# bronemos/view-fusion

Measured on AMD Instinct MI355X. Metric: denoise_steps_per_sec, higher is better.
Workload: dtype f32; 1 GPU; small UNet 64x64 (33.9M params), B=16/GPU N=6 (S=96 views/GPU), training iteration fwd+bwd+Adam, linear T=2000 schedule; global_batch=16, views=6, parallelism=dp1, launch=HIP-graph replay of the whole iteration

## Files before the change

include/vf_hip.h:

```cpp
#ifndef VF_HIP_H
#define VF_HIP_H
#ifdef __cplusplus
extern "C" {
#endif

int vf_gn_fwd(const float* x, const float* gamma, const float* beta, float* y, float* mean ,
              float* rstd , int S, int C, int HW, int groups, float eps, int silu, void* stream);
int vf_gn_bwd_emits_rowsum(int C, int HW, int groups);
int vf_gn_plan(int C, int HW, int groups, int cat, int C1, int has_addend, int has_addend2, int has_dx2, int* out );
int vf_gn_bwd(const float* x, const float* gamma, const float* beta, const float* mean, const float* rstd,
              const float* dy, const float* addend, float* dx, float* dgamma_part, float* dbeta_part,
              float* dx_rowsum, int S, int C, int HW, int groups, int silu, void* stream);
int vf_gn_cat_fwd(const float* x, const float* x2, int C1, const float* gamma, const float* beta, float* y, float* mean,
                  float* rstd, int S, int C, int HW, int groups, float eps, int silu, void* stream);
int vf_gn_cat_bwd(const float* x, const float* x2, int C1, const float* gamma, const float* beta, const float* mean,
                  const float* rstd, const float* dy, const float* addend, const float* addend2, float* dx, float* dx2,
                  float* dgamma_part, float* dbeta_part, float* dx_rowsum, int S, int C, int HW, int groups, int silu,
                  void* stream);
int vf_rowsum(const float* x, float* out , int rows, int len, void* stream);
int vf_bias_grad(const float* dy, float* db, float* dvb, int S, int C, int HW, void* stream);
int vf_colsum(const float* part , float* out , int batch, int S, int C,
              void* stream);
int vf_colsum_multi(const void* desc, int n, long total_blocks, void* stream);

// ... 39 lines not shown
                         long ws_floats, int S, int Cin, int Cout, int H, int W, void* stream);
long vf_conv1x1_bf16x3_pack_dwords(int M, int K);
int vf_conv1x1_bf16x3_pack(const float* w_oihw, void* w3_fwd, void* w3_bwd, int Cout, int Cin, void* stream);
int vf_conv1x1_bf16x3(const float* x, const float* x2, int C1in, const void* w3, const float* bias,
                      const float* view_bias, const float* residual, float* y, float* y2, int C1out, int S, int Cin,
                      int Cout, int HW, void* stream);
long vf_conv_wgrad_ws_floats(int S, int Cin, int Cout, int H, int W, int KS);
int vf_conv_wgrad(const float* x, const float* dy, float* dw_oihw, float* ws, long ws_floats, int S, int Cin,
                  int Cout, int H, int W, int KS, int mode, void* stream);
int vf_conv_wgrad_main(const float* x, const float* dy, float* dw_oihw, float* ws, long ws_floats, int S, int Cin,
                       int Cout, int H, int W, int KS, int mode, long long* desc9, int* nblocks, void* stream);
int vf_conv1x1_cat_wgrad_main(const float* x1, const float* x2, int C1, const float* dy, float* dw_oihw, float* ws,
                              long ws_floats, int S, int Cin, int Cout, int H, int W, long long* desc9, int* nblocks,
                              void* stream);
int vf_sumpool2(const float* x, float* y, long n_out, int Wo, void* stream);

int vf_wino_supported(int H, int W, int mode);
int vf_wino_pack_sizes(int Cout, int Cin, long* fwd_floats, long* bwd_floats);
int vf_wino_pack_weights(const float* w_oihw, float* u_fwd, float* u_bwd , int Cout, int Cin,
                         void* stream);
int vf_wino_pack_weights_multi(const void* desc, int nlayers, long total_blocks, void* stream);
long vf_wino_conv_ws_floats(int S, int Cin, int Cout, int H, int W);
int vf_wino_conv_fill_pct(int S, int Cin, int Cout, int H, int W, int* tiles_out);
int vf_wino_conv_fwd(const float* x, const float* u_packed, const float* bias, const float* view_bias,
                     const float* residual, float* y, float* ws, long ws_floats, int S, int Cin, int Cout, int H,
                     int W, int mode, void* stream);
int vf_wino_conv_gn_fusable(int S, int Cin, int Cout, int H, int W, int mode, int groups);
int vf_wino_conv_fwd_gn(const float* x, const float* u_packed, const float* bias , const float* view_bias ,
                        const float* residual , float* y, int store_y, const float* gn_gamma, const float* gn_beta,
                        float* a_out, int groups, float eps, int silu, float* ws, long ws_floats, int S, int Cin, int Cout,
// ... 272 lines not shown
```

view_fusion_amd/_lib.py:

```python
import ctypes
import os

import torch

_HERE = os.path.dirname(os.path.abspath(__file__))
LIB_PATH = os.path.join(_HERE, "lib", "libvf_hip.so")
_OVERRIDE = os.environ.get("VF_HIP_LIB") if os.environ.get("VF_DEBUG_AB") == "1" else None
if _OVERRIDE:
    LIB_PATH = _OVERRIDE
elif os.environ.get("VF_HIP_LIB"):
    import warnings
    warnings.warn("VF_HIP_LIB is ignored unless VF_DEBUG_AB=1 (kernel-tuning aid)", stacklevel=2)

_P, _I, _L, _F = ctypes.c_void_p, ctypes.c_int, ctypes.c_long, ctypes.c_float
_U64 = ctypes.c_uint64

SIGNATURES = {
    "vf_gn_fwd": [_P, _P, _P, _P, _P, _P, _I, _I, _I, _I, _F, _I, _P],
    "vf_gn_bwd_emits_rowsum": [_I, _I, _I],
    "vf_gn_plan": [_I, _I, _I, _I, _I, _I, _I, _I, _P],
    "vf_gn_cat_fwd": [_P, _P, _I, _P, _P, _P, _P, _P, _I, _I, _I, _I, _F, _I, _P],
    "vf_gn_cat_bwd": [_P, _P, _I, _P, _P, _P, _P, _P, _P, _P, _P, _P, _P, _P, _P, _I, _I, _I, _I, _I, _P],
    "vf_conv1x1_cat_fwd": [_P, _P, _I, _P, _P, _P, _P, _L, _I, _I, _I, _I, _I, _P],
    "vf_conv1x1_cat_dgrad": [_P, _P, _P, _P, _I, _I, _I, _I, _I, _I, _P],
# ... 28 lines not shown
    "vf_wino44_pack_sizes": [_I, _I, ctypes.POINTER(_L), ctypes.POINTER(_L)],
    "vf_wino44_pack_weights": [_P, _P, _P, _I, _I, _P],
    "vf_wino44_pack_weights_multi": [_P, _I, _L, _P],
    "vf_wino44_conv_ws_floats": [_I, _I, _I, _I, _I],
    "vf_wino44_conv_fill_pct": [_I, _I, _I, _I, _I, ctypes.POINTER(_I)],
    "vf_wino44_conv_fwd": [_P, _P, _P, _P, _P, _P, _P, _L, _I, _I, _I, _I, _I, _I, _P],
    "vf_wino_conv_plan": [_I, _I, _I, _I, _I, _I, _I, _I, _L, _P],
    "vf_wino_wgrad_ws_floats": [_I, _I, _I, _I, _I],
    "vf_wino_wgrad_supported": [_I, _I, _I],
    "vf_wino_wgrad": [_P, _P, _P, _P, _P, _P, _L, _I, _I, _I, _I, _I, _I, _P],
    "vf_wino_wgrad_main": [_P, _P, _P, _P, _P, _P, _L, _I, _I, _I, _I, _I, _I, _P, _P, _P],
    "vf_wino44_reduce_multi": [_P, _I, _I, _P],
    "vf_conv_wgrad_main": [_P, _P, _P, _P, _L, _I, _I, _I, _I, _I, _I, _I, _P, _P, _P],
    "vf_conv1x1_cat_wgrad_main": [_P, _P, _I, _P, _P, _P, _L, _I, _I, _I, _I, _I, _P, _P, _P],
    "vf_sumpool2": [_P, _P, _L, _I, _P],
    "vf_time_affine_fwd": [_P, _I, _P, _P, _I, _I, _I, _P],
    "vf_time_affine_ws_floats": [_I, _I],
    "vf_time_affine_bwd": [_P, _I, _P, _P, _P, _P, _P, _P, _P, _I, _I, _I, _P],
    "vf_bgemm": [_P, _P, _P, _P, _I, _I, _I, _I, _L, _L, _L, _L, _L, _L, _L, _L, _L, _F, _F, _P],
    "vf_attention_fwd": [_P, _P, _P, _I, _I, _I, _P],
    "vf_attention_fwd_kernel": [_I, _I, _I],
    "vf_attention_dscore": [_P, _P, _P, _P, _P, _I, _I, _I, _P],
    "vf_attention_dvdk": [_P, _P, _P, _P, _P, _I, _I, _I, _P],
    "vf_attn_stream_fwd": [_P, _P, _P, _I, _I, _I, _P],
    "vf_attn_stream_bwd": [_P, _P, _P, _P, _P, _P, _I, _I, _I, _P],
    "vf_attn_stream_plan": [_P, _P, _I, _I, _I, _P],
    "vf_softmax_fwd": [_P, _P, _I, _I, _P],
    "vf_softmax_bwd": [_P, _P, _P, _I, _I, _P],
    "vf_bgemm_plan": [_P, _P, _I, _I, _I, _I, _L, _L, _L, _L, _L, _L, _L, _P],
    "vf_softmax_plan": [_I, _I, _P],
# ... 83 lines not shown
    "vf_distill_target": [_P, _P, _P, _P, _P, _P, _P, _P, _P, _P, _P, _P, _P, _P, _I, _I, _I, _I, _P, _P],
    "vf_distill_step_host": [_U64, _P, _I, _P, _I],
    "vf_loss_weights_trunc_snr_host": [_P, _I, _I, _P],
    "vf_stack_views_sc": [_P, _P, _P, _P, _P, _P, _P, _P, _P, _P, _P, _I, _I, _I, _I, _I, _I, _I, _P],
    "vf_draw_self_cond": [_U64, _P, ctypes.c_uint, _P, _I, _P],
    "vf_self_cond_estimate": [_P, _P, _P, _P, _L, _L, _I, _P, _P, _I, _I, _I, _I, _I, _P],
    "vf_self_cond_draw_host": [_U64, _P, ctypes.c_uint, _P, _I],
    "vf_self_cond_coeffs_host": [_P, _I, _P, _P, _I],
    "vf_rng_host_philox": [_P, _P, _P],
    "vf_rng_host_normal": [_U64, _P, _I, _I, _P, _I, _I],
    "vf_rng_host_train_scalars": [_U64, _P, _I, _P, _P, _I],
    "vf_batch_assemble": [_P, _L, _I, _I, _U64, _P, _P, _I, _I, _I, _I, _P, _P, _P, _P, _P],
    "vf_batch_host_plan": [_U64, _P, _I, _I, _I, _I, _L, _P, _P, _P, _P, _P, _P, _P],
}
_RESTYPE = {"vf_conv1x1_bf16x3_pack_dwords": _L, "vf_conv_wgrad_ws_floats": _L, "vf_time_affine_ws_floats": _L, "vf_wino_conv_ws_floats": _L, "vf_wino44_conv_ws_floats": _L, "vf_wino_wgrad_ws_floats": _L, "vf_conv_fwd_ws_floats": _L,
            "vf_conv_small_pack_floats": _L, "vf_ssim_workspace_floats": _L, "vf_lpips_workspace_floats": _L}

_lib = None
N_CALLS = 0


class VFHipError(RuntimeError):
    pass


def load():
    global _lib
    if _lib is None:
        if not os.path.exists(LIB_PATH):
            raise VFHipError(
                f"{LIB_PATH} not found: build it with `python -m view_fusion_amd.build` "
# ... 23 lines not shown
```

view_fusion_amd/ops/conv.py:

```python
import ctypes

import torch

from .. import _lib, reducer
from .state import st
from .bf16x3 import _packed_b3, _use_b3
from .core import _MODES, _c, _call, _check, _launch, _ptr, _stream, _workspace
from .deferred import _defer_begin, _gout, _rowsum_get, _rowsum_put, _wred_ws
from .norm import group_norm
from .packing import _WINO_ABI, _conv_ws, _packed, _packed_small, _packed_wino, _wino_ws
from .policy import use_small_conv, use_winograd, use_winograd_wgrad, wino_kind


def _wgrad(entry, front, back, need, owners, keep, generic, flops, tag, strm):
    dev = keep[0].device
    ws = _wred_ws(dev, need) if (st.WRED_DEFER and (st.WRED_DEFER_GENERIC or not generic)
                                 and _defer_begin(owners, st.slab_sums)) else None
    if ws is None:
        ws = _workspace(dev, need)
        _launch("conv_wgrad", flops, entry, *front, _ptr(ws), ws.numel(), *back, strm, tag=tag)
        return False
    row, nblk = (ctypes.c_longlong * 9)(), ctypes.c_int(0)
    _launch("conv_wgrad", flops, entry + "_main", *front, _ptr(ws), ws.numel(), *back, ctypes.cast(row, ctypes.c_void_p),
            ctypes.cast(ctypes.pointer(nblk), ctypes.c_void_p), strm, tag=tag)
    st.slab_sums.add(dev, (list(row), nblk.value, (ws, *keep)))
    return True


def _conv_small(x, x2, weight, bias, view_bias, residual, S, Cin, Cout, H, W, KS, m):
    wd = weight.detach()
    _check(wd)
    y = torch.empty(S, Cout, H, W, device=x.device, dtype=torch.float32)
    wp = _packed_small(weight) if KS == 3 else None
    if wp is not None:
        _launch("conv_fwd", 2.0 * S * Cout * Cin * 9 * H * W, "vf_conv_small_gn", _ptr(x), None, 0, _ptr(wd), _ptr(bias),
                _ptr(view_bias), _ptr(residual), _ptr(y), S, Cin, Cout, H, W, 3, None, None, None, 0, 1e-5, 0, None, None,
                None, 0, 0, None, None, _ptr(wp), m, _stream(), tag=(Cin, Cout, H, KS, m))
        return y
    _launch("conv_fwd", 2.0 * S * Cout * Cin * KS * KS * H * W, "vf_conv_small", _ptr(x), _ptr(x2),
            x.shape[1] if x2 is not None else 0, _ptr(wd), _ptr(bias), _ptr(view_bias), _ptr(residual), _ptr(y), S, Cin,
            Cout, H, W, KS, m, _stream(), tag=(Cin, Cout, H, KS, m))
# ... 28 lines not shown
        _check(x, bias, view_bias, residual)
        ctx.tap = tap
        if tap:
            ctx.set_materialize_grads(False)
        S, Cin, Hi, Wi = x.shape
        Cout, _, KS, _ = weight.shape
        m = _MODES[mode]
        if m == 1 and (Hi % 2 or Wi % 2):
            raise ValueError(f"stride-2 conv on a {Hi}x{Wi} map: both sides must be even")
        H, W = (Hi // 2, Wi // 2) if m == 1 else ((Hi * 2, Wi * 2) if m == 2 else (Hi, Wi))
        y = torch.empty(S, Cout, H, W, device=x.device, dtype=torch.float32)
        flops = 2.0 * S * Cout * Cin * KS * KS * H * W
        nb = 4.0 * (x.numel() + y.numel() + weight.numel() + (residual.numel() if residual is not None else 0))
        wino = wino_kind(S, Cin, Cout, H, W, KS, m, train=bool(training))
        ctx.b3 = _use_b3(KS, m, H * W)
        if ctx.b3:
            wf, wb = _packed_b3(layer, force=training)
            _launch("conv_fwd", flops, "vf_conv1x1_bf16x3", _ptr(x), None, 0, ctypes.c_void_p(wf.data_ptr()), _ptr(bias),
                    _ptr(view_bias), _ptr(residual), _ptr(y), None, 0, S, Cin, Cout, H * W, _stream(),
                    tag=(Cin, Cout, H, KS, m))
        elif wino:
            wf, wb = _packed_wino(layer, training, wino)
            ws, nws = _wino_ws(x.device, S, Cin, Cout, H, W, wino)
            _launch("conv_fwd", flops, _WINO_ABI[wino][3], _ptr(x), _ptr(wf), _ptr(bias), _ptr(view_bias),
                    _ptr(residual), _ptr(y), _ptr(ws), nws, S, Cin, Cout, H, W, m, _stream(),
                    tag=(Cin, Cout, H, KS, m), nbytes=nb)
        else:
            wf, wb = _packed(layer, force=training)
            ws, nws = _conv_ws(x.device, S, Cin, Cout, H, W, KS)
            _launch("conv_fwd", flops, "vf_conv_fwd", _ptr(x), _ptr(wf), _ptr(bias), _ptr(view_bias),
                    _ptr(residual), _ptr(y), _ptr(ws), nws, S, Cin, Cout, H, W, KS, m, _stream(),
# ... 4 lines not shown
        ctx.wb, ctx.m, ctx.KS, ctx.Cout = wb, m, KS, Cout
        ctx.has = (bias is not None, view_bias is not None, residual is not None)
        ctx.pw, ctx.pb, ctx.twin = weight, bias, (twin.bias if twin is not None else None)
        return (y, x.view_as(x)) if tap else y

    @staticmethod
    def backward(ctx, dy, dtap=None):
        (x,) = ctx.saved_tensors
        dy = _c(dy)
        dtap = _c(dtap) if dtap is not None else None
        S, Cin, Hi, Wi = x.shape
        _, Cout, H, W = dy.shape
        KS, m = ctx.KS, ctx.m
        strm = _stream()
        dx = dw = db = dvb = dres = None
        if ctx.needs_input_grad[0] and ctx.wino:
            dfull = torch.empty(S, Cin, H, W, device=x.device, dtype=torch.float32)
            ws, nws = _wino_ws(x.device, S, Cout, Cin, H, W, ctx.wino)
            _launch("conv_dgrad", ctx.flops, _WINO_ABI[ctx.wino][3], _ptr(dy), _ptr(ctx.wb), None, None, None,
                    _ptr(dfull), _ptr(ws), nws, S, Cout, Cin, H, W, 0, strm, tag=ctx.tag,
                    nbytes=4.0 * (dy.numel() + dfull.numel() + ctx.pw.numel()))
            if m == 2:
                dx = torch.empty_like(x)
                _call("vf_sumpool2", _ptr(dfull), _ptr(dx), dx.numel(), Wi, strm)
            else:
                dx = dfull
        elif ctx.needs_input_grad[0] and ctx.b3:
            dx = torch.empty_like(x)
            _launch("conv_dgrad", ctx.flops, "vf_conv1x1_bf16x3", _ptr(dy), None, 0, ctypes.c_void_p(ctx.wb.data_ptr()), None,
                    None, None, _ptr(dx), None, 0, S, Cout, Cin, H * W, strm, tag=ctx.tag)
        elif ctx.needs_input_grad[0]:
# ... 8 lines not shown
                        None, 0, S, Cout, Cin, H, W, KS, 4, strm, tag=ctx.tag)
                dtap = None
            else:
                dup = torch.empty(S, Cin, H, W, device=x.device, dtype=torch.float32)
                _launch("conv_dgrad", ctx.flops, "vf_conv_fwd", _ptr(dy), _ptr(ctx.wb), None, None, None, _ptr(dup),
                        None, 0, S, Cout, Cin, H, W, KS, 0, strm, tag=ctx.tag)
                dx = torch.empty_like(x)
                _call("vf_sumpool2", _ptr(dup), _ptr(dx), dx.numel(), Wi, strm)
        hb, hv, hr = ctx.has
        want_b, want_v = hb and ctx.needs_input_grad[2], hv and ctx.needs_input_grad[3]
        arena = reducer.ACTIVE is not None
        hit = _rowsum_get(dy) if (want_b or want_v) else None
        if hit is not None:
            dvb, db = hit[1], (hit[2].view_as(hit[2]) if hit[2] is not None else None)
        db2 = None
        if ctx.needs_input_grad[1] and use_winograd_wgrad(S, Cin, Cout, H, W, KS, m):
            need = _lib.load().vf_wino_wgrad_ws_floats(S, Cin, Cout, H, W)
            dw = _gout(ctx.pw, Cout, Cin, 3, 3, like=x)
            db_here = None
            if want_b and db is None:
                db = db_here = _gout(ctx.pb, Cout, like=x)
                if hr:
                    db2 = _gout(ctx.twin, Cout, like=x)
            owners = [ctx.pw] + ([ctx.pb] if db_here is not None else []) + \
                     ([ctx.twin] if (db2 is not None and ctx.twin is not None) else [])
            if _wgrad("vf_wino_wgrad", (_ptr(x), _ptr(dy), _ptr(dw), _ptr(db_here), _ptr(db2)), (S, Cin, Cout, H, W, m),
                      need, owners, (dw, db_here, db2), False, ctx.flops, ctx.tag, strm):
                dw = dw.view_as(dw)
                if db_here is not None:
                    db = db_here.view_as(db_here)
        elif ctx.needs_input_grad[1]:
# ... 159 lines not shown
```

view_fusion_amd/ops/state.py:

```python
import os


class State:
    def __init__(self):
        self.KERNEL_LOG = None
        self._KIND_OVERRIDE = None
        self.WINOGRAD = True
        self.FORCE_WINOGRAD = False
        self.WINO_MIN_TILES = int(os.environ.get("VF_WINO_MIN_TILES", 30))
        self.WINO_MIN_FILL = int(os.environ.get("VF_WINO_MIN_FILL", 65))
        self.WINO_WGRAD_MIN_TILES = int(os.environ.get("VF_WINO_WGRAD_MIN_TILES", 256))
        self.WINOGRAD_WGRAD = True
        self.WINOGRAD44 = os.environ.get("VF_WINO44", "1") == "1"
        self.FORCE_WINOGRAD44 = False
        self.SMALL_CONV = os.environ.get("VF_SMALL_CONV", "1") == "1"
        self.SMALL_CONV_MAX_WGS = (int(os.environ.get("VF_SMALL_CONV_MAX_WGS1", 1024)),
                          int(os.environ.get("VF_SMALL_CONV_MAX_WGS3", 512)))
        self.SMALL_CONV_MAX_CIN3 = int(os.environ.get("VF_SMALL_CONV_MAX_CIN3", 256))
        self.SMALL_CONV_MAX_S3 = int(os.environ.get("VF_SMALL_CONV_MAX_S3", 1))
        self.SMALL_PACK = os.environ.get("VF_SMALL_PACK", "1") == "1"
        self.RES_FOLD = os.environ.get("VF_RES_FOLD", "1") == "1"
        self.WINO_GN_FUSION = os.environ.get("VF_WINO_GN", "1") == "1"
        self.ATTN_DSCORE = os.environ.get("VF_ATTN_DSCORE", "1") != "0"
        self.ATTN_DVDK = os.environ.get("VF_ATTN_DVDK", "1") != "0"
        self.BF16X3 = os.environ.get("VF_BF16X3") == "1"
        self.ROWSUM_FUSION = True
        self.COLSUM_DEFER = True
        self.WRED_DEFER = os.environ.get("VF_WRED_DEFER", "1") != "0"
        self.WRED_DEFER_GENERIC = os.environ.get("VF_WRED_DEFER_GENERIC", "1") != "0"
# ... 15 lines not shown
```

view_fusion_amd/train.py:

```python
import contextlib
import math
import os

import torch
import torch.distributed as dist
from torch.nn.parallel import DistributedDataParallel

from . import reducer
from .unet import UNet
from .view_fusion import ViewFusion

SMALL_UNET = dict(in_channel=6, out_channel=6, inner_channel=64, norm_groups=32, channel_mults=(1, 2, 3, 5),
                  attn_res=(16,), res_blocks=3, image_size=64)
BETA_SCHEDULE = {
    "train": dict(schedule="linear", num_timesteps=2000, linear_start=1e-6, linear_end=1e-2),
    "test": dict(schedule="linear", num_timesteps=1000, linear_start=1e-4, linear_end=0.09),
}


class LrScheduler:

    def __init__(self, peak_lr=1e-4, peak_it=2500, decay_rate=0.16, decay_it=4000000):
        self.peak_lr, self.peak_it, self.decay_rate, self.decay_it = peak_lr, peak_it, decay_rate, decay_it

# ... 298 lines not shown
            return False
        acc = self.opt.accum_begin() if accum else None
        if accum and acc is None:
            return False
        if self._scal is None:
            self._scal = torch.zeros(3, device=dev, dtype=torch.float32)
        e.inputs = {k: {**batch, **extra}[k].detach().clone().contiguous() for k, _, _ in key[:-2]}
        e.view_count = torch.tensor(vc, dtype=torch.int64, device=dev)
        offs = ops.view_offsets(e.view_count, dev)
        e.off, e.vc = offs[0], vc
        tables = ops.prime_tables(getattr(self.module, "denoise_fn", None), key[-1], dev, tuple(batch["y_0"].shape[-2:]))
        self.opt.zero_grad()
        g = torch.cuda.CUDAGraph()
        kw = {} if self._pool is None else dict(pool=self._pool)
        ops.begin_capture(dev, sum(1 for m in self.module.modules() if isinstance(m, torch.nn.GroupNorm)),
                          sum(1 for m in self.module.modules() if isinstance(m, torch.nn.Conv2d)))
        failed = None
        try:
            with torch.cuda.graph(g, capture_error_mode="relaxed", **kw):
                try:
                    leaves = {n: p.detach().requires_grad_(True) for n, p in self._named}
                    if arena is not None:
                        arena.capture_begin(list(leaves.values()))
                    seeded = {} if extra.get("seed") is None else dict(seed=extra["seed"])
                    loss = torch.func.functional_call(self.model, leaves, (),
                                                      dict(view_count=e.view_count, **e.inputs, **seeded))
                    grads = torch.autograd.grad(loss, list(leaves.values()), allow_unused=True)
                    if arena is not None:
                        grads = arena.capture_finish(grads)
                    for (_, p), gr in zip(self._named, grads):
                        p.grad = gr
# ... 167 lines not shown
```

view_fusion_amd/unet.py:

```python
import torch
from torch import nn


class _Named(nn.Module):

    def __init__(self, **children):
        super().__init__()
        for name, mod in children.items():
            self.add_module(name, mod)

    def __getitem__(self, name):
        return self._modules[name]


def _norm_act_conv(cin, cout, groups):
    return _Named(block=_Named(**{"0": nn.GroupNorm(groups, cin), "3": nn.Conv2d(cin, cout, 3, padding=1)}))


class _ResBlock(nn.Module):
    def __init__(self, cin, cout, emb_dim, groups, dropout=0):
        super().__init__()
        self.noise_func = _Named(noise_func=_Named(**{"0": nn.Linear(emb_dim, cout)}))
        self.block1 = _norm_act_conv(cin, cout, groups)
        self.block2 = _norm_act_conv(cout, cout, groups)
# ... 185 lines not shown
                mark_block(layer, lvl)
            elif isinstance(layer, _Resample):
                lvl += 1
                mark(layer.conv, lvl, "down2")
            else:
                mark(layer, lvl)
        for layer in self.mid:
            mark_block(layer, lvl)
        for layer in self.ups:
            if isinstance(layer, _ResAttnBlock):
                mark_block(layer, lvl)
            else:
                lvl -= 1
                mark(layer.conv, lvl, "up2")
        mark(self.final_conv["block"]["3"], lvl)
        object.__setattr__(self, "_vf_image_size", image_size)
        object.__setattr__(self, "_vf_depth", sum(isinstance(m, _Resample) and not m.up for m in self.downs))
        object.__setattr__(self, "_vf_attn_levels", tuple(sorted(attn_levels)))

    def check_input_size(self, H, W):
        f = 1 << self._vf_depth
        if H <= 0 or W <= 0 or H % f or W % f:
            raise ValueError(f"input size {H}x{W}: both sides must be positive multiples of {f} "
                             f"(2**(len(channel_mults) - 1)) for the encoder / decoder maps to match")
        if (H * W) % 4:
            raise ValueError(f"input size {H}x{W}: H*W must be a multiple of 4")

    def _affine_layers(self):
        lst = getattr(self, "_vf_affine", None)
        if lst is None:
# ... 92 lines not shown
```

Baseline: 3271 view denoise-steps/s (UNet fwd+bwd per stacked view, incl. compose/MSE/Adam).

## Add dedicated narrow-channel 3x3 conv kernels for UNet first and final convs

Adds specialized HIP kernels for 3x3 convolutions where one side has at most 8 channels (the UNet input conv and final output conv). They cover the forward pass, the transposed dgrad, and a weight-gradient kernel that also accumulates the bias gradient. The forward and wgrad kernels use MFMA f32 with LDS halo strips, and the output-narrow path uses per-wave FMA with a cross-wave reduction. This replaces the Winograd path, which wastes work when the channel count is tiny. The cost is added code complexity and an extra wgrad slab-reduction row per narrow layer.

```diff
diff --git a/include/vf_hip.h b/include/vf_hip.h
--- a/include/vf_hip.h
+++ b/include/vf_hip.h
@@ -77,6 +77,15 @@
                               long ws_floats, int S, int Cin, int Cout, int H, int W, long long* desc9, int* nblocks,
                               void* stream);
 int vf_sumpool2(const float* x, float* y, long n_out, int Wo, void* stream);
+
+int vf_conv_narrow_kind(int Cin, int Cout, int H, int W);
+int vf_conv_narrow_fwd(const float* x, const float* w_oihw, int transposed, const float* bias, const float* view_bias,
+                       const float* residual, float* y, int S, int Cin, int Cout, int H, int W, void* stream);
+long vf_conv_narrow_wgrad_ws_floats(int S, int Cin, int Cout, int H, int W);
+int vf_conv_narrow_wgrad(const float* x, const float* dy, float* dw_oihw, float* db, float* ws, long ws_floats, int S,
+                         int Cin, int Cout, int H, int W, void* stream);
+int vf_conv_narrow_wgrad_main(const float* x, const float* dy, float* dw_oihw, float* db, float* ws, long ws_floats, int S,
+                              int Cin, int Cout, int H, int W, long long* desc18, int* nblocks2, void* stream);
 
 int vf_wino_supported(int H, int W, int mode);
 int vf_wino_pack_sizes(int Cout, int Cin, long* fwd_floats, long* bwd_floats);
diff --git a/view_fusion_amd/_lib.py b/view_fusion_amd/_lib.py
--- a/view_fusion_amd/_lib.py
+++ b/view_fusion_amd/_lib.py
@@ -66,6 +66,11 @@
     "vf_conv_wgrad_main": [_P, _P, _P, _P, _L, _I, _I, _I, _I, _I, _I, _I, _P, _P, _P],
     "vf_conv1x1_cat_wgrad_main": [_P, _P, _I, _P, _P, _P, _L, _I, _I, _I, _I, _I, _P, _P, _P],
     "vf_sumpool2": [_P, _P, _L, _I, _P],
+    "vf_conv_narrow_kind": [_I, _I, _I, _I],
+    "vf_conv_narrow_fwd": [_P, _P, _I, _P, _P, _P, _P, _I, _I, _I, _I, _I, _P],
+    "vf_conv_narrow_wgrad_ws_floats": [_I, _I, _I, _I, _I],
+    "vf_conv_narrow_wgrad": [_P, _P, _P, _P, _P, _L, _I, _I, _I, _I, _I, _P],
+    "vf_conv_narrow_wgrad_main": [_P, _P, _P, _P, _P, _L, _I, _I, _I, _I, _I, _P, _P, _P],
     "vf_time_affine_fwd": [_P, _I, _P, _P, _I, _I, _I, _P],
     "vf_time_affine_ws_floats": [_I, _I],
     "vf_time_affine_bwd": [_P, _I, _P, _P, _P, _P, _P, _P, _P, _I, _I, _I, _P],
@@ -179,7 +184,7 @@
     "vf_batch_host_plan": [_U64, _P, _I, _I, _I, _I, _L, _P, _P, _P, _P, _P, _P, _P],
 }
 _RESTYPE = {"vf_conv1x1_bf16x3_pack_dwords": _L, "vf_conv_wgrad_ws_floats": _L, "vf_time_affine_ws_floats": _L, "vf_wino_conv_ws_floats": _L, "vf_wino44_conv_ws_floats": _L, "vf_wino_wgrad_ws_floats": _L, "vf_conv_fwd_ws_floats": _L,
-            "vf_conv_small_pack_floats": _L, "vf_ssim_workspace_floats": _L, "vf_lpips_workspace_floats": _L}
+            "vf_conv_narrow_wgrad_ws_floats": _L, "vf_conv_small_pack_floats": _L,"vf_ssim_workspace_floats": _L, "vf_lpips_workspace_floats": _L}
 
 _lib = None
 N_CALLS = 0
diff --git a/view_fusion_amd/csrc/conv_narrow.hip b/view_fusion_amd/csrc/conv_narrow.hip
--- /dev/null
+++ b/view_fusion_amd/csrc/conv_narrow.hip
@@ -0,0 +1,513 @@
+#include "common.h"
+#include "wgrad_reduce.h"
+
+namespace {
+
+constexpr int TWM = 64;
+constexpr int PITCH = TWM + 8;
+
+struct NarrowArgs {
+    const float* x;
+    const float* w;
+    const float* bias;
+    const float* vbias;
+    const float* res;
+    float* y;
+    int S, Cin, Cout, H, W, transposed, tiles_x, tiles_y;
+};
+
+__device__ __forceinline__ void keep(float& v) { asm volatile("" : "+v"(v)); }
+__device__ __forceinline__ void keep(f32x4& v) { asm volatile("" : "+v"(v)); }
+
+__device__ __forceinline__ float plane_near(const float* __restrict__ p, int gy, int gx, int H, int W) {
+    return p[(size_t)min(max(gy, 0), H - 1) * W + min(max(gx, 0), W - 1)];
+}
+__device__ __forceinline__ bool inside(int gy, int gx, int H, int W) { return gy >= 0 && gy < H && gx >= 0 && gx < W; }
+
+template <int TH, int MAXCH, int NT>
+struct HaloStrip {
+    static constexpr int PER = (TH + 2) * (TWM + 2), NIT = (MAXCH * PER + NT - 1) / NT;
+    float v[NIT];
+    __device__ __forceinline__ void load(const float* __restrict__ src, int nch, int y0, int x0, int H, int W, int tid) {
+        const int total = nch * PER;
+#pragma unroll
+        for (int j = 0; j < NIT; ++j) {
+            const int i = min(tid + NT * j, total - 1);
+            const int ci = i / PER, rem = i % PER, r = rem / (TWM + 2), cc = rem % (TWM + 2);
+            v[j] = plane_near(src + (size_t)ci * H * W, y0 - 1 + r, x0 - 1 + cc, H, W);
+        }
+    }
+    template <int CHS>
+    __device__ __forceinline__ void store(float* lds, int nch, int y0, int x0, int tw, int H, int W, int tid) {
+        const int total = nch * PER;
+#pragma unroll
+        for (int j = 0; j < NIT; ++j) keep(v[j]);
+#pragma unroll
+        for (int j = 0; j < NIT; ++j) {
+            const int i = tid + NT * j;
+            if (i < total) {
+                const int ci = i / PER, rem = i % PER, r = rem / (TWM + 2), cc = rem % (TWM + 2);
+                lds[ci * CHS + r * PITCH + 3 + cc] = (cc <= tw + 1 && inside(y0 - 1 + r, x0 - 1 + cc, H, W)) ? v[j] : 0.f;
+            }
+        }
+    }
+};
+
+constexpr int NI_TH = 4;
+constexpr int NI_CH = (NI_TH + 2) * PITCH;
+
+template <int CIN>
+__global__ __launch_bounds__(256, 2) void narrow_in_kernel(const NarrowArgs a) {
+    constexpr int K = 9 * CIN, KP = (K + 1) / 2, ZS = CIN * NI_CH;
+    __shared__ float xs[CIN * NI_CH + 4];
+    const int tid = threadIdx.x, lane = tid & 63, wave = tid >> 6, half = lane >> 5, l32 = lane & 31;
+    const int H = a.H, W = a.W, Cout = a.Cout, ntiles = a.S * a.tiles_x * a.tiles_y;
+    auto origin = [&](int t, int& s, int& y0, int& x0) {
+        x0 = (t % a.tiles_x) * TWM; t /= a.tiles_x;
+        y0 = (t % a.tiles_y) * NI_TH; s = t / a.tiles_y;
+    };
+    HaloStrip<NI_TH, CIN, 256> strip;
+    int s, y0, x0;
+    origin(min((int)blockIdx.x, ntiles - 1), s, y0, x0);
+    strip.load(a.x + (size_t)s * CIN * H * W, CIN, y0, x0, H, W, tid);
+    if (tid < 4) xs[ZS + tid] = 0.f;
+    float wv[KP], badd[16];
+    int cur_mt = -1;
+  for (int t = blockIdx.x; t < ntiles; t += gridDim.x) {
+    origin(t, s, y0, x0);
+    const int tw = min(TWM, W - x0), qpr = tw >> 2, nq = NI_TH * qpr;
+    int tid_ = tid;
+    asm volatile("" : "+v"(tid_));
+    if (t != (int)blockIdx.x) __syncthreads();
+    strip.template store<NI_CH>(xs, CIN, y0, x0, tw, H, W, tid_);
+    __syncthreads();
+    if (t + (int)gridDim.x < ntiles) {
+        int s2, y2, x2;
+        origin(t + gridDim.x, s2, y2, x2);
+        strip.load(a.x + (size_t)s2 * CIN * H * W, CIN, y2, x2, H, W, tid_);
+    }
+
+    const int nblk = (nq + 31) >> 5, nmt = (Cout + 31) >> 5;
+    for (int item = wave; item < nblk * nmt; item += 4) {
+        const int blk = item % nblk, mt = item / nblk;
+        const int g = blk * 32 + l32;
+        const bool valid = g < nq;
+        const int gg = valid ? g : 0, r = gg / qpr, c4 = gg % qpr;
+        const int base = r * PITCH + 3 + 4 * c4;
+        const int co = mt * 32 + l32;
+        if (mt != cur_mt) {
+            cur_mt = mt;
+#pragma unroll
+            for (int kk = 0; kk < KP; ++kk) {
+                const int k = min(2 * kk + half, K - 1), cc = min(co, Cout - 1);
+                const int wi = a.transposed ? ((k / 9) * Cout + cc) * 9 + 8 - k % 9 : cc * K + k;
+                wv[kk] = a.w[wi];
+            }
+#pragma unroll
+            for (int kk = 0; kk < KP; ++kk) keep(wv[kk]);
+#pragma unroll
+            for (int kk = 0; kk < KP; ++kk)
+                if (!(co < Cout && 2 * kk + half < K)) wv[kk] = 0.f;
+#pragma unroll
+            for (int v = 0; v < 16; ++v)
+                badd[v] = a.bias ? a.bias[min(mt * 32 + 8 * (v >> 2) + 4 * half + (v & 3), Cout - 1)] : 0.f;
+        }
+        f32x16 acc[4];
+#pragma unroll
+        for (int v = 0; v < 16; ++v) {
+            float t = badd[v];
+            if (a.vbias) t += a.vbias[(size_t)s * Cout + min(mt * 32 + 8 * (v >> 2) + 4 * half + (v & 3), Cout - 1)];
+#pragma unroll
+            for (int q = 0; q < 4; ++q) acc[q][v] = t;
+        }
+#pragma unroll
+        for (int kk = 0; kk < KP; ++kk) {
+            const int k0 = 2 * kk, k1 = 2 * kk + 1;
+            const int o0 = (k0 / 9) * NI_CH + ((k0 % 9) / 3) * PITCH + (k0 % 9) % 3;
+            const int o1 = (k1 / 9) * NI_CH + ((k1 % 9) / 3) * PITCH + (k1 % 9) % 3;
+            const int addr = half ? (k1 < K ? base + o1 : ZS) : base + o0;
+#pragma unroll
+            for (int q = 0; q < 4; ++q)
+                acc[q] = __builtin_amdgcn_mfma_f32_32x32x2f32(wv[kk], xs[addr + q], acc[q], 0, 0, 0);
+        }
+        const int oy = y0 + r;
+        if (valid && oy < H) {
+#pragma unroll
+            for (int v = 0; v < 16; ++v) {
+                const int c = mt * 32 + 8 * (v >> 2) + 4 * half + (v & 3);
+                if (c < Cout) {
+                    const size_t o = (((size_t)s * Cout + c) * H + oy) * W + x0 + 4 * c4;
+                    f32x4 out = {acc[0][v], acc[1][v], acc[2][v], acc[3][v]};
+                    if (a.res) out += *reinterpret_cast<const f32x4*>(a.res + o);
+                    *reinterpret_cast<f32x4*>(a.y + o) = out;
+                }
+            }
+        }
+    }
+  }
+}
+
+constexpr int NO_TH = 4, NO_CK = 4;
+constexpr int NO_CH = (NO_TH + 2) * PITCH;
+constexpr int NO_WAVE = NO_CK * NO_CH;
+
+template <int NO, bool TR>
+__global__ __launch_bounds__(256, 4) void narrow_out_kernel(const NarrowArgs a) {
+    __shared__ __attribute__((aligned(16))) float xs[4 * NO_WAVE];
+    static_assert(3 * NO * 4 * 64 <= 4 * NO_WAVE, "the partial sums of waves 1..3 fit the staging area");
+    const int tid = threadIdx.x, lane = tid & 63, wave = tid >> 6;
+    int b = blockIdx.x;
+    const int tx = b % a.tiles_x; b /= a.tiles_x;
+    const int ty = b % a.tiles_y;
+    const int s = b / a.tiles_y;
+    const int x0 = tx * TWM, y0 = ty * NO_TH, H = a.H, W = a.W, Cin = a.Cin;
+    const int tw = min(TWM, W - x0), qpr = tw >> 2, nq = NO_TH * qpr;
+    const bool valid = lane < nq;
+    const int gg = valid ? lane : 0, r = gg / qpr, c4 = gg % qpr;
+    const float* __restrict__ w = a.w;
+    const int sc = TR ? NO * 9 : 9, so = TR ? 9 : Cin * 9;
+    float* my = xs + wave * NO_WAVE;
+
+    float acc[NO][4];
+#pragma unroll
+    for (int o = 0; o < NO; ++o)
+#pragma unroll
+        for (int q = 0; q < 4; ++q) acc[o][q] = 0.f;
+
+    for (int c0 = wave * NO_CK; c0 < Cin; c0 += 4 * NO_CK) {
+        const float* __restrict__ xv = a.x + ((size_t)s * Cin + c0) * H * W;
+        constexpr int NV = NO_CK * (NO_TH + 2) * (TWM / 4) / 64;
+        f32x4 v[NV];
+#pragma unroll
+        for (int j = 0; j < NV; ++j) {
+            const int i = lane + 64 * j;
+            const int ci = i / ((NO_TH + 2) * (TWM / 4)), rem = i % ((NO_TH + 2) * (TWM / 4));
+            const int rr = rem / (TWM / 4), q4 = rem % (TWM / 4), gy = y0 - 1 + rr;
+            v[j] = *reinterpret_cast<const f32x4*>(xv + ((size_t)ci * H + min(max(gy, 0), H - 1)) * W + x0 +
+                                                   4 * min(q4, qpr - 1));
+        }
+        const int hl = min(lane, NO_CK * (NO_TH + 2) * 2 - 1);
+        const int hci = hl / ((NO_TH + 2) * 2), hrem = hl % ((NO_TH + 2) * 2), hrr = hrem >> 1, hcc = (hrem & 1) ? tw : -1;
+        float hv = plane_near(xv + (size_t)hci * H * W, y0 - 1 + hrr, x0 + hcc, H, W);
+#pragma unroll
+        for (int j = 0; j < NV; ++j) keep(v[j]);
+        keep(hv);
+        if (!inside(y0 - 1 + hrr, x0 + hcc, H, W)) hv = 0.f;
+#pragma unroll
+        for (int j = 0; j < NV; ++j) {
+            const int i = lane + 64 * j, rem = i % ((NO_TH + 2) * (TWM / 4)), gy = y0 - 1 + rem / (TWM / 4);
+            if (!(gy >= 0 && gy < H && rem % (TWM / 4) < qpr)) v[j] = f32x4{0.f, 0.f, 0.f, 0.f};
+        }
+        __builtin_amdgcn_wave_barrier();
+#pragma unroll
+        for (int j = 0; j < NV; ++j) {
+            const int i = lane + 64 * j;
+            const int ci = i / ((NO_TH + 2) * (TWM / 4)), rem = i % ((NO_TH + 2) * (TWM / 4));
+            *reinterpret_cast<f32x4*>(&my[ci * NO_CH + (rem / (TWM / 4)) * PITCH + 4 + 4 * (rem % (TWM / 4))]) = v[j];
+        }
+        __builtin_amdgcn_wave_barrier();
+        if (lane < NO_CK * (NO_TH + 2) * 2) my[hci * NO_CH + hrr * PITCH + 4 + hcc] = hv;
+        __builtin_amdgcn_fence(__ATOMIC_RELEASE, "wavefront");
+        __builtin_amdgcn_wave_barrier();
+        __builtin_amdgcn_fence(__ATOMIC_ACQUIRE, "wavefront");
+#pragma unroll 1
+        for (int ci = 0; ci < NO_CK; ++ci) {
+            const float* __restrict__ wc = w + (size_t)(c0 + ci) * sc;
+#pragma unroll
+            for (int dy = 0; dy < 3; ++dy) {
+                const float* p = &my[ci * NO_CH + (r + dy) * PITCH + 4 * c4 + 3];
+                const f32x4 m = *reinterpret_cast<const f32x4*>(p + 1);
+                const float in[6] = {p[0], m[0], m[1], m[2], m[3], p[5]};
+#pragma unroll
+                for (int dx = 0; dx < 3; ++dx)
+#pragma unroll
+                    for (int o = 0; o < NO; ++o) {
+                        const float wv = wc[o * so + (TR ? 8 - (dy * 3 + dx) : dy * 3 + dx)];
+#pragma unroll
+                        for (int q = 0; q < 4; ++q) acc[o][q] = fmaf(wv, in[q + dx], acc[o][q]);
+                    }
+            }
+        }
+    }
+    __syncthreads();
+    if (wave) {
+#pragma unroll
+        for (int o = 0; o < NO; ++o)
+#pragma unroll
+            for (int q = 0; q < 4; ++q) xs[(((wave - 1) * NO + o) * 4 + q) * 64 + lane] = acc[o][q];
+    }
+    __syncthreads();
+    const int oy = y0 + r;
+    if (wave == 0 && valid && oy < H) {
+#pragma unroll
+        for (int o = 0; o < NO; ++o) {
+#pragma unroll
+            for (int q = 0; q < 4; ++q)
+#pragma unroll
+                for (int ww = 0; ww < 3; ++ww) acc[o][q] += xs[((ww * NO + o) * 4 + q) * 64 + lane];
+            float add = a.bias ? a.bias[o] : 0.f;
+            if (a.vbias) add += a.vbias[(size_t)s * NO + o];
+            const size_t off = (((size_t)s * NO + o) * H + oy) * W + x0 + 4 * c4;
+            f32x4 out = {acc[o][0] + add, acc[o][1] + add, acc[o][2] + add, acc[o][3] + add};
+            if (a.res) out += *reinterpret_cast<const f32x4*>(a.res + off);
+            *reinterpret_cast<f32x4*>(a.y + off) = out;
+        }
+    }
+}
+
+constexpr int WG_TH = 2;
+constexpr int WG_CS = WG_TH * TWM + 1;
+constexpr int WG_NCH = (WG_TH + 2) * PITCH + 3;
+constexpr int WG_NV = 64 * WG_TH * (TWM / 4) / 256;
+
+struct NarrowWgradArgs {
+    const float* wide;
+    const float* narrow;
+    float* ws;
+    float* bsum;
+    int S, Cw, Cn, H, W, flip, tiles_x, tiles_y, ntiles;
+};
+
+struct WgTile { int s, x0, y0, tw; };
+
+__device__ __forceinline__ WgTile wg_tile(const NarrowWgradArgs& a, int t) {
+    WgTile r;
+    const int tx = t % a.tiles_x; t /= a.tiles_x;
+    r.s = t / a.tiles_y; r.y0 = (t % a.tiles_y) * WG_TH; r.x0 = tx * TWM; r.tw = min(TWM, a.W - r.x0);
+    return r;
+}
+
+__device__ __forceinline__ void wg_load_wide(const NarrowWgradArgs& a, const WgTile& t, int w0, int cwg, int tid, f32x4* v) {
+    const float* __restrict__ wv = a.wide + ((size_t)t.s * a.Cw + w0) * a.H * a.W;
+    const int qpr = t.tw >> 2;
+#pragma unroll
+    for (int j = 0; j < WG_NV; ++j) {
+        const int i = tid + 256 * j;
+        const int c = i / (WG_TH * (TWM / 4)), rem = i % (WG_TH * (TWM / 4)), r = rem / (TWM / 4), q4 = rem % (TWM / 4);
+        v[j] = *reinterpret_cast<const f32x4*>(wv + ((size_t)min(c, cwg - 1) * a.H + min(t.y0 + r, a.H - 1)) * a.W +
+                                               t.x0 + 4 * min(q4, qpr - 1));
+    }
+}
+
+__global__ __launch_bounds__(256, 2) void narrow_wgrad_kernel(const NarrowWgradArgs a) {
+    constexpr int NAR = 8 * WG_NCH;
+    __shared__ float wl[64 * WG_CS];
+    __shared__ float nl[NAR + 2];
+    const int tid = threadIdx.x, lane = tid & 63, wave = tid >> 6, half = lane >> 5, l32 = lane & 31;
+    const int Cw = a.Cw, Cn = a.Cn, H = a.H, W = a.W;
+    const int w0 = blockIdx.y * 64, cwg = min(64, Cw - w0);
+    const int ncol = 9 * Cn, ncolb = ncol + ((a.flip || !a.bsum) ? 0 : 1);
+    const int nmt = (cwg + 31) >> 5, nnt = (ncolb + 31) >> 5, nitems = nmt * nnt;
+
+    int abase[2], bbase[2], bmove[2];
+    f32x16 acc[2];
+#pragma unroll
+    for (int it = 0; it < 2; ++it) {
+        const int item = wave + 4 * it, mt = item % nmt, nt = item / nmt;
+        abase[it] = (mt * 32 + l32) * WG_CS;
+        const int j = nt * 32 + l32;
+        if (j < ncol) {
+            const int tap = j / Cn, n = j % Cn, te = a.flip ? 8 - tap : tap;
+            bbase[it] = n * WG_NCH + (te / 3) * PITCH + 3 + te % 3;
+            bmove[it] = 1;
+        } else {
+            bbase[it] = NAR + (j == ncol && ncolb > ncol ? 1 : 0);
+            bmove[it] = 0;
+        }
+#pragma unroll
+        for (int v = 0; v < 16; ++v) acc[it][v] = 0.f;
+    }
+    if (tid == 0) { nl[NAR] = 0.f; nl[NAR + 1] = 1.f; }
+    float bacc = 0.f;
+
+    f32x4 pre[WG_NV];
+    HaloStrip<WG_TH, 8, 256> strip;
+    {
+        const WgTile t0 = wg_tile(a, min((int)blockIdx.x, a.ntiles - 1));
+        wg_load_wide(a, t0, w0, cwg, tid, pre);
+        strip.load(a.narrow + (size_t)t0.s * Cn * H * W, Cn, t0.y0, t0.x0, H, W, tid);
+    }
+    for (int t = blockIdx.x; t < a.ntiles; t += gridDim.x) {
+        const WgTile tl = wg_tile(a, t);
+        const int tw = tl.tw;
+        if (t != (int)blockIdx.x) __syncthreads();
+#pragma unroll
+        for (int j = 0; j < WG_NV; ++j) keep(pre[j]);
+#pragma unroll
+        for (int j = 0; j < WG_NV; ++j) {
+            const int i = tid + 256 * j, c = i / (WG_TH * (TWM / 4)), rem = i % (WG_TH * (TWM / 4));
+            const bool ok = c < cwg && tl.y0 + rem / (TWM / 4) < H && rem % (TWM / 4) < (tw >> 2);
+            float* d = &wl[c * WG_CS + rem * 4];
+            d[0] = ok ? pre[j][0] : 0.f; d[1] = ok ? pre[j][1] : 0.f; d[2] = ok ? pre[j][2] : 0.f; d[3] = ok ? pre[j][3] : 0.f;
+        }
+        strip.template store<WG_NCH>(nl, Cn, tl.y0, tl.x0, tw, H, W, tid);
+        __syncthreads();
+        if (t + (int)gridDim.x < a.ntiles) {
+            const WgTile tn = wg_tile(a, t + gridDim.x);
+            wg_load_wide(a, tn, w0, cwg, tid, pre);
+            strip.load(a.narrow + (size_t)tn.s * Cn * H * W, Cn, tn.y0, tn.x0, H, W, tid);
+        }
+        if (a.flip && a.bsum && (tid >> 5) < Cn) {
+            const float* p = &nl[(tid >> 5) * WG_NCH + PITCH + 4];
+#pragma unroll
+            for (int i = 0; i < WG_TH * TWM / 32; ++i) {
+                const int px = l32 + 32 * i;
+                bacc += p[(px / TWM) * PITCH + px % TWM];
+            }
+        }
+#pragma unroll
+        for (int it = 0; it < 2; ++it) {
+            if (wave + 4 * it < nitems) {
+                for (int r = 0; r < WG_TH; ++r) {
+                    const float* pa = &wl[abase[it] + r * TWM + half];
+                    const float* pb = &nl[bbase[it] + bmove[it] * (r * PITCH + half)];
+                    const int step = 2 * bmove[it];
+                    float a0 = pa[0], a1 = pa[2], b0 = pb[0], b1 = pb[step];
+                    for (int x = 4; x < tw; x += 4) {
+                        pb += 2 * step;
+                        const float n0 = pa[x], n1 = pa[x + 2], m0 = pb[0], m1 = pb[step];
+                        acc[it] = __builtin_amdgcn_mfma_f32_32x32x2f32(a0, b0, acc[it], 0, 0, 0);
+                        acc[it] = __builtin_amdgcn_mfma_f32_32x32x2f32(a1, b1, acc[it], 0, 0, 0);
+                        a0 = n0; a1 = n1; b0 = m0; b1 = m1;
+                    }
+                    acc[it] = __builtin_amdgcn_mfma_f32_32x32x2f32(a0, b0, acc[it], 0, 0, 0);
+                    acc[it] = __builtin_amdgcn_mfma_f32_32x32x2f32(a1, b1, acc[it], 0, 0, 0);
+                }
+            }
+        }
+    }
+
+    const int Cout = a.flip ? Cn : Cw, Cin = a.flip ? Cw : Cn;
+    float* __restrict__ slab = a.ws + (size_t)blockIdx.x * 9 * Cout * Cin;
+#pragma unroll
+    for (int it = 0; it < 2; ++it) {
+        const int item = wave + 4 * it, mt = item % nmt, nt = item / nmt;
+        if (item < nitems) {
+            const int j = nt * 32 + l32;
+#pragma unroll
+            for (int v = 0; v < 16; ++v) {
+                const int i = mt * 32 + 8 * (v >> 2) + 4 * half + (v & 3);
+                if (i < cwg) {
+                    const int cw = w0 + i;
+                    if (j < ncol) {
+                        const int tap = j / Cn, n = j % Cn;
+                        slab[a.flip ? ((size_t)tap * Cout + n) * Cin + cw : ((size_t)tap * Cout + cw) * Cin + n] = acc[it][v];
+                    } else if (j == ncol && ncolb > ncol) {
+                        a.bsum[(size_t)blockIdx.x * Cout + cw] = acc[it][v];
+                    }
+                }
+            }
+        }
+    }
+    if (a.flip && a.bsum && blockIdx.y == 0) {
+        const float t = seg_sum<32>(bacc);
+        if (l32 == 0 && (tid >> 5) < Cn) a.bsum[(size_t)blockIdx.x * Cout + (tid >> 5)] = t;
+    }
+}
+
+__global__ __launch_bounds__(256) void narrow_reduce_kernel(const W44Red rw, const W44Red rb) {
+    const int bid = blockIdx.x;
+    if (bid < rw.nmain) wgrad_reduce_body(rw.ws, rw.dw, rw.nslab, rw.nt, rw.Cout, rw.Cin, rw.CoutP, rw.CinQ, bid);
+    else wgrad_reduce_body(rb.ws, rb.dw, rb.nslab, rb.nt, rb.Cout, rb.Cin, rb.CoutP, rb.CinQ, bid - rw.nmain);
+}
+
+constexpr int WGRAD_MAX_SLABS = 512;
+
+inline int ceil_div(int a, int b) { return (a + b - 1) / b; }
+
+inline int narrow_kind(int Cin, int Cout, int H, int W) {
+    if (H <= 0 || W <= 0 || W % 4 != 0 || Cin <= 0 || Cout <= 0) return 0;
+    if (Cin <= 8 && Cout % 16 == 0) return 1;
+    if (Cout <= 8 && Cin % 8 == 0) return 2;
+    return 0;
+}
+
+inline int wgrad_slabs(int S, int H, int W) {
+    const long nt = (long)S * ceil_div(H, WG_TH) * ceil_div(W, TWM);
+    return (int)(nt < WGRAD_MAX_SLABS ? nt : WGRAD_MAX_SLABS);
+}
+
+int narrow_wgrad_impl(const float* x, const float* dy, float* dw, float* db, float* ws, long ws_floats, int S, int Cin,
+                      int Cout, int H, int W, hipStream_t st, long long* desc, int* nblocks) {
+    if (desc) nblocks[0] = nblocks[1] = 0;
+    const int flip = Cout <= 8 ? 1 : 0;
+    const int Cw = flip ? Cin : Cout, Cn = flip ? Cout : Cin;
+    if (!narrow_kind(Cin, Cout, H, W) || Cn > 8 || Cw % 16 != 0 || !x || !dy || !dw || !ws) return (int)hipErrorInvalidValue;
+    if (S <= 0) return 0;
+    const int z = wgrad_slabs(S, H, W);
+    const size_t slab = (size_t)9 * Cout * Cin;
+    if ((size_t)ws_floats < (size_t)z * (slab + Cout)) return (int)hipErrorInvalidValue;
+    NarrowWgradArgs a;
+    a.wide = flip ? x : dy; a.narrow = flip ? dy : x; a.ws = ws; a.bsum = db ? ws + (size_t)z * slab : nullptr;
+    a.S = S; a.Cw = Cw; a.Cn = Cn; a.H = H; a.W = W; a.flip = flip;
+    a.tiles_x = ceil_div(W, TWM); a.tiles_y = ceil_div(H, WG_TH); a.ntiles = S * a.tiles_x * a.tiles_y;
+    hipLaunchKernelGGL(narrow_wgrad_kernel, dim3(z, ceil_div(Cw, 64)), dim3(256), 0, st, a);
+    long long rows[18];
+    const int nw = wgrad_reduce_row(rows, ws, dw, z, 9, Cout, Cin, Cout, Cin);
+    const int nb = db ? wgrad_reduce_row(rows + 9, a.bsum, db, z, 1, Cout, 1, Cout, 1) : 0;
+    if (desc) {
+        memcpy(desc, rows, (db ? 18 : 9) * sizeof(long long));
+        nblocks[0] = nw; nblocks[1] = nb;
+        VF_RETURN_LAST_ERROR();
+    }
+    W44Red rw, rb;
+    memcpy(&rw, rows, sizeof rw);
+    if (db) memcpy(&rb, rows + 9, sizeof rb); else rb = rw;
+    hipLaunchKernelGGL(narrow_reduce_kernel, dim3(nw + nb), dim3(256), 0, st, rw, rb);
+    VF_RETURN_LAST_ERROR();
+}
+
+template <int C>
+int launch_narrow(int kind, const NarrowArgs& a, hipStream_t st) {
+    const dim3 grid(a.S * a.tiles_x * a.tiles_y);
+    if (kind == 1) hipLaunchKernelGGL((narrow_in_kernel<C>), dim3(grid.x < 512u ? grid.x : 512u), dim3(256), 0, st, a);
+    else if (a.transposed) hipLaunchKernelGGL((narrow_out_kernel<C, true>), grid, dim3(256), 0, st, a);
+    else hipLaunchKernelGGL((narrow_out_kernel<C, false>), grid, dim3(256), 0, st, a);
+    VF_RETURN_LAST_ERROR();
+}
+
+}
+
+extern "C" {
+
+int vf_conv_narrow_kind(int Cin, int Cout, int H, int W) { return narrow_kind(Cin, Cout, H, W); }
+
+int vf_conv_narrow_fwd(const float* x, const float* w_oihw, int transposed, const float* bias, const float* view_bias,
+                       const float* residual, float* y, int S, int Cin, int Cout, int H, int W, void* stream) {
+    const int kind = narrow_kind(Cin, Cout, H, W);
+    if (!kind || !x || !w_oihw || !y) return (int)hipErrorInvalidValue;
+    if (S <= 0) return 0;
+    NarrowArgs a;
+    a.x = x; a.w = w_oihw; a.bias = bias; a.vbias = view_bias; a.res = residual; a.y = y;
+    a.S = S; a.Cin = Cin; a.Cout = Cout; a.H = H; a.W = W; a.transposed = transposed ? 1 : 0;
+    a.tiles_x = ceil_div(W, TWM); a.tiles_y = ceil_div(H, kind == 1 ? NI_TH : NO_TH);
+    hipStream_t st = (hipStream_t)stream;
+    switch (kind == 1 ? Cin : Cout) {
+        case 1: return launch_narrow<1>(kind, a, st);
+        case 2: return launch_narrow<2>(kind, a, st);
+        case 3: return launch_narrow<3>(kind, a, st);
+        case 4: return launch_narrow<4>(kind, a, st);
+        case 5: return launch_narrow<5>(kind, a, st);
+        case 6: return launch_narrow<6>(kind, a, st);
+        case 7: return launch_narrow<7>(kind, a, st);
+        default: return launch_narrow<8>(kind, a, st);
+    }
+}
+
+long vf_conv_narrow_wgrad_ws_floats(int S, int Cin, int Cout, int H, int W) {
+    if (S <= 0 || !narrow_kind(Cin, Cout, H, W)) return 0;
+    return (long)wgrad_slabs(S, H, W) * ((long)9 * Cout * Cin + Cout);
+}
+
+int vf_conv_narrow_wgrad(const float* x, const float* dy, float* dw, float* db, float* ws, long ws_floats, int S, int Cin,
+                         int Cout, int H, int W, void* stream) {
+    return narrow_wgrad_impl(x, dy, dw, db, ws, ws_floats, S, Cin, Cout, H, W, (hipStream_t)stream, nullptr, nullptr);
+}
+
+int vf_conv_narrow_wgrad_main(const float* x, const float* dy, float* dw, float* db, float* ws, long ws_floats, int S,
+                              int Cin, int Cout, int H, int W, long long* desc18, int* nblocks2, void* stream) {
+    if (!desc18 || !nblocks2) return (int)hipErrorInvalidValue;
+    return narrow_wgrad_impl(x, dy, dw, db, ws, ws_floats, S, Cin, Cout, H, W, (hipStream_t)stream, desc18, nblocks2);
+}
+
+}
diff --git a/view_fusion_amd/ops/conv.py b/view_fusion_amd/ops/conv.py
--- a/view_fusion_amd/ops/conv.py
+++ b/view_fusion_amd/ops/conv.py
@@ -12,7 +12,7 @@
 from .policy import use_small_conv, use_winograd, use_winograd_wgrad, wino_kind
 
 
-def _wgrad(entry, front, back, need, owners, keep, generic, flops, tag, strm):
+def _wgrad(entry, front, back, need, owners, keep, generic, flops, tag, strm, nrows=1):
     dev = keep[0].device
     ws = _wred_ws(dev, need) if (st.WRED_DEFER and (st.WRED_DEFER_GENERIC or not generic)
                                  and _defer_begin(owners, st.slab_sums)) else None
@@ -20,11 +20,21 @@
         ws = _workspace(dev, need)
         _launch("conv_wgrad", flops, entry, *front, _ptr(ws), ws.numel(), *back, strm, tag=tag)
         return False
-    row, nblk = (ctypes.c_longlong * 9)(), ctypes.c_int(0)
+    row, nblk = (ctypes.c_longlong * (9 * nrows))(), (ctypes.c_int * nrows)()
     _launch("conv_wgrad", flops, entry + "_main", *front, _ptr(ws), ws.numel(), *back, ctypes.cast(row, ctypes.c_void_p),
-            ctypes.cast(ctypes.pointer(nblk), ctypes.c_void_p), strm, tag=tag)
-    st.slab_sums.add(dev, (list(row), nblk.value, (ws, *keep)))
+            ctypes.cast(nblk, ctypes.c_void_p), strm, tag=tag)
+    for i in range(nrows):
+        if i == 0 or nblk[i]:
+            st.slab_sums.add(dev, (list(row[9 * i:9 * i + 9]), nblk[i], (ws, *keep)))
     return True
+
+
+def _narrow_route(layer, twin, S, Cin, Cout, H, W, KS, m, wino):
+    if not (st.NARROW_CONV and wino and KS == 3 and m == 0 and twin is None and getattr(layer, "_vf_narrow", False)):
+        return False
+    lib = _lib.load()
+    return bool(min(Cin, Cout) <= 8 and max(Cin, Cout) % 16 == 0 and lib.vf_conv_narrow_kind(Cin, Cout, H, W)
+                and lib.vf_conv_narrow_kind(Cout, Cin, H, W))
 
 
 def _conv_small(x, x2, weight, bias, view_bias, residual, S, Cin, Cout, H, W, KS, m):
@@ -83,7 +93,13 @@
         nb = 4.0 * (x.numel() + y.numel() + weight.numel() + (residual.numel() if residual is not None else 0))
         wino = wino_kind(S, Cin, Cout, H, W, KS, m, train=bool(training))
         ctx.b3 = _use_b3(KS, m, H * W)
-        if ctx.b3:
+        ctx.narrow = not ctx.b3 and _narrow_route(layer, twin, S, Cin, Cout, H, W, KS, m, wino)
+        wb = None
+        if ctx.narrow:
+            _check(weight.detach())
+            _launch("conv_fwd", flops, "vf_conv_narrow_fwd", _ptr(x), _ptr(weight), 0, _ptr(bias), _ptr(view_bias),
+                    _ptr(residual), _ptr(y), S, Cin, Cout, H, W, _stream(), tag=(Cin, Cout, H, KS, m), nbytes=nb)
+        elif ctx.b3:
             wf, wb = _packed_b3(layer, force=training)
             _launch("conv_fwd", flops, "vf_conv1x1_bf16x3", _ptr(x), None, 0, ctypes.c_void_p(wf.data_ptr()), _ptr(bias),
                     _ptr(view_bias), _ptr(residual), _ptr(y), None, 0, S, Cin, Cout, H * W, _stream(),
@@ -118,7 +134,11 @@
         KS, m = ctx.KS, ctx.m
         strm = _stream()
         dx = dw = db = dvb = dres = None
-        if ctx.needs_input_grad[0] and ctx.wino:
+        if ctx.needs_input_grad[0] and ctx.narrow:
+            dx = torch.empty_like(x)
+            _launch("conv_dgrad", ctx.flops, "vf_conv_narrow_fwd", _ptr(dy), _ptr(ctx.pw), 1, None, None, None, _ptr(dx),
+                    S, Cout, Cin, H, W, strm, tag=ctx.tag, nbytes=4.0 * (dy.numel() + dx.numel() + ctx.pw.numel()))
+        elif ctx.needs_input_grad[0] and ctx.wino:
             dfull = torch.empty(S, Cin, H, W, device=x.device, dtype=torch.float32)
             ws, nws = _wino_ws(x.device, S, Cout, Cin, H, W, ctx.wino)
             _launch("conv_dgrad", ctx.flops, _WINO_ABI[ctx.wino][3], _ptr(dy), _ptr(ctx.wb), None, None, None,
@@ -157,7 +177,19 @@
         if hit is not None:
             dvb, db = hit[1], (hit[2].view_as(hit[2]) if hit[2] is not None else None)
         db2 = None
-        if ctx.needs_input_grad[1] and use_winograd_wgrad(S, Cin, Cout, H, W, KS, m):
+        if ctx.needs_input_grad[1] and ctx.narrow:
+            need = _lib.load().vf_conv_narrow_wgrad_ws_floats(S, Cin, Cout, H, W)
+            dw = _gout(ctx.pw, Cout, Cin, 3, 3, like=x)
+            db_here = None
+            if want_b and db is None:
+                db = db_here = _gout(ctx.pb, Cout, like=x)
+            if _wgrad("vf_conv_narrow_wgrad", (_ptr(x), _ptr(dy), _ptr(dw), _ptr(db_here)), (S, Cin, Cout, H, W), need,
+                      [ctx.pw] + ([ctx.pb] if db_here is not None else []), (dw, db_here, None), True, ctx.flops, ctx.tag,
+                      strm, nrows=2):
+                dw = dw.view_as(dw)
+                if db_here is not None:
+                    db = db_here.view_as(db_here)
+        elif ctx.needs_input_grad[1] and use_winograd_wgrad(S, Cin, Cout, H, W, KS, m):
             need = _lib.load().vf_wino_wgrad_ws_floats(S, Cin, Cout, H, W)
             dw = _gout(ctx.pw, Cout, Cin, 3, 3, like=x)
             db_here = None
diff --git a/view_fusion_amd/ops/state.py b/view_fusion_amd/ops/state.py
--- a/view_fusion_amd/ops/state.py
+++ b/view_fusion_amd/ops/state.py
@@ -13,6 +13,7 @@
         self.WINOGRAD_WGRAD = True
         self.WINOGRAD44 = os.environ.get("VF_WINO44", "1") == "1"
         self.FORCE_WINOGRAD44 = False
+        self.NARROW_CONV = os.environ.get("VF_NARROW_CONV", "1") == "1"
         self.SMALL_CONV = os.environ.get("VF_SMALL_CONV", "1") == "1"
         self.SMALL_CONV_MAX_WGS = (int(os.environ.get("VF_SMALL_CONV_MAX_WGS1", 1024)),
                           int(os.environ.get("VF_SMALL_CONV_MAX_WGS3", 512)))
diff --git a/view_fusion_amd/train.py b/view_fusion_amd/train.py
--- a/view_fusion_amd/train.py
+++ b/view_fusion_amd/train.py
@@ -336,7 +336,8 @@
         g = torch.cuda.CUDAGraph()
         kw = {} if self._pool is None else dict(pool=self._pool)
         ops.begin_capture(dev, sum(1 for m in self.module.modules() if isinstance(m, torch.nn.GroupNorm)),
-                          sum(1 for m in self.module.modules() if isinstance(m, torch.nn.Conv2d)))
+                          sum(1 + bool(getattr(m, "_vf_narrow", False)) for m in self.module.modules()
+                              if isinstance(m, torch.nn.Conv2d)))
         failed = None
         try:
             with torch.cuda.graph(g, capture_error_mode="relaxed", **kw):
diff --git a/view_fusion_amd/unet.py b/view_fusion_amd/unet.py
--- a/view_fusion_amd/unet.py
+++ b/view_fusion_amd/unet.py
@@ -223,6 +223,8 @@
                 lvl -= 1
                 mark(layer.conv, lvl, "up2")
         mark(self.final_conv["block"]["3"], lvl)
+        for conv in (self.downs[0], self.final_conv["block"]["3"]):
+            object.__setattr__(conv, "_vf_narrow", True)
         object.__setattr__(self, "_vf_image_size", image_size)
         object.__setattr__(self, "_vf_depth", sum(isinstance(m, _Resample) and not m.up for m in self.downs))
         object.__setattr__(self, "_vf_attn_levels", tuple(sorted(attn_levels)))
```

After: 3281 view denoise-steps/s (UNet fwd+bwd per stacked view, incl. compose/MSE/Adam), median of 6. Within noise of the previous version (+0.3%).
